# timwhite0/smcdet

Measured on AMD Instinct MI355X. Metric: particle-steps/sec (4096 particles, 32x32 tile), higher is better.
Workload: dtype f32

## Files before the change

smcdet_amd/csrc/mh_kernel.hip:

```cpp
#include <math.h>
#include <string.h>

#include <algorithm>
#include <cmath>
#include <mutex>
#include <type_traits>
#include <vector>

#include "mh_plan.h"
#include "render.h"
#include "tile.h"

namespace smcdet {

SMCDET_WAVE_TABLE

#ifdef SMCDET_DIAG
constexpr bool kDiag = true;
#else
constexpr bool kDiag = false;
#endif

constexpr int kMhBlock = kMhWaves * kWave;
constexpr int kSlots = 6;
constexpr int kBatch = 21;

struct MhArgs {
  DevModel m;
  DevPrior pr;
  int K, T, N, S;
  float sl, isl, sf, isf;
  float lb_h, lb_w, ub_h, ub_w;
  float lb_f, ub_f;
  uint32_t k0, k1;
  uint64_t offset;
  uint32_t ablate;
  int by_count;
  int scalar_slots;
  int skip_done;
  int no_psf_cache;
  int no_rcp_cache;
  int blk_slots;
  int generic_geometry;
  int no_write_through;
  int write_through;
  const float4* psf_tab;
  float tab_inv_h;
  const float* img;
  const float* temperature;
  const int64_t* ancestors;
  const float* anc_bins;
  const float* counts_in;
  const float* locs_in;
  const float* fluxes_in;
  float* counts_out;
  float* locs_out;
  float* fluxes_out;
  float* loglik_out;
  const float* rate_in;
  float* rate_out;
  const int32_t* go;
  const float* boxes;
  int32_t* acc_count;
  float* acc_rate;
  const int32_t* r_comp;
  const float* r_uloc;
  const float* r_uflux;
  const float* r_uacc;
  float* r_loga;
  uint8_t* r_accept;
  int has_tail;
  TileArgs tail;
};

constexpr int kTailMaxN = 8 * kTB;
static_assert(kMhPad == kWave && kMhMaxLdsPixels == kMaxLdsPixels && kMhTailMaxN == kTailMaxN &&
                  kMhTabFloats * sizeof(float) == kTabNodes * sizeof(float4),
              "mh_plan.h: constants out of step with device.h / tile.h");

__device__ __forceinline__ void tn_cache(float mu, float isig, float lb, float ub, float& phl,
                                         float& lZ) {
  phl = normal_cdf(lb, mu, isig);
  lZ = nan_to_num(fast_log(normal_cdf(ub, mu, isig) - phl), 0.0f);
}

__device__ __forceinline__ bool edge_hit(float hast) { return __float_as_uint(hast) == 0xff800000u; }

struct Proposal {
  int j;
  float h, w;
  float hn, wn, fn;
  float hast;
};

struct Dim {
  float sig, isig, lb, ub;
};

template <bool ABLATE>
__device__ __forceinline__ void propose_lane(float mu, float c_ph, float c_lZ, float u,
                                             const Dim& dm, float& xn, float& n_ph, float& n_lZ,
                                             float& hast_d, float& n_lf) {
  if (ABLATE) {
    xn = fminf(fmaxf(mu + (u - 0.5f) * dm.sig, dm.lb), dm.ub);
    n_ph = c_ph;
    n_lZ = c_lZ;
    hast_d = 0.f;
    n_lf = xn;
  } else {
    const float pc = fminf(fmaxf(u, 1e-6f), 0.999999f);
    float pt = c_ph + pc * fast_exp(c_lZ);
    pt = fminf(fmaxf(pt, 1e-6f), 0.999999f);
    xn = mu + dm.sig * erfinv_fast(2.0f * pt - 1.0f) * kSqrt2;
    xn = fminf(fmaxf(xn, dm.lb), dm.ub);
    tn_cache(xn, dm.isig, dm.lb, dm.ub, n_ph, n_lZ);
    hast_d = c_lZ - n_lZ;
    n_lf = fast_log(xn);
  }
}

template <int MODEL, bool WINDOWS, bool GL = false, bool RV = false, bool TB = false>
__device__ __forceinline__ float position_delta(const DevModel& m, const float* xs,
                                                const float* lg, const float* lam,
                                                const float* rv, const float4* tab, float tinv,
                                                int p, int aa, int bb, int ph, int pw,
                                                const Proposal& P, float amp_o, float amp_n,
                                                int ao_h, int ao_w, int an_h, int an_w,
                                                float& lnew, float& rnew) {
  const float fph = (float)ph + 0.5f, fpw = (float)pw + 0.5f;
  const float dho = fph - P.h, dwo = fpw - P.w;
  const float dhn = fph - P.hn, dwn = fpw - P.wn;
  float psi_o, psi_n;
  if constexpr (TB) {
    psi_o = psf_tab(tab, tinv, fmaf(dho, dho, dwo * dwo));
    psi_n = psf_tab(tab, tinv, fmaf(dhn, dhn, dwn * dwn));
  } else {
    psi_o = psf_raw<MODEL>(m, fmaf(dho, dho, dwo * dwo));
    psi_n = psf_raw<MODEL>(m, fmaf(dhn, dhn, dwn * dwn));
  }
  if (WINDOWS) {
    const unsigned span = 2u * (unsigned)m.R;
    psi_o = ((unsigned)(aa - ao_h) <= span && (unsigned)(bb - ao_w) <= span) ? psi_o : 0.f;
    psi_n = ((unsigned)(aa - an_h) <= span && (unsigned)(bb - an_w) <= span) ? psi_n : 0.f;
  }
  const float dl = fmaf(amp_n, psi_n, -amp_o * psi_o);
  const float lo = lam[p];
  lnew = lo + dl;
  const float lgx = (MODEL == SMCDET_MODEL_POISSON) ? lg[p] : 0.0f;
  const float x = GL ? xs[min(p, m.H * m.W - 1)] : xs[p];
  if constexpr (RV) {
    const float r0 = rv[p];
    const float v1 = fmaf(m.eta, lnew, m.s0sq);
    const float r1 = fast_rcp(v1);
    rnew = r1;
    const float d0 = x - lo, d1 = x - lnew;
    const float t = fmaf(d0 * d0, r0, -(d1 * d1) * r1);
    return fmaf(0.5f, t, (-0.5f * kLn2) * fast_log2(v1 * r0));
  }
  return pix_delta<MODEL>(m, x, lgx, lo, dl);
}

template <int MODEL, bool WINDOWS, bool GL = false, bool RV = false, bool TB = false>
__device__ __forceinline__ f2 position_delta2(const DevModel& m, const float* xs, const float* lg,
                                             const float* lam, const float* rv,
                                             const float4* tab, float tinv, const int (&p)[2],
                                             const int (&aa)[2], const int (&bb)[2], f2 fph,
                                             f2 fpw, const Proposal& P, float amp_o, float amp_n,
                                             int ao_h, int ao_w, int an_h, int an_w, f2& lnew,
                                             f2& rnew) {
  const f2 dho = fph - P.h, dwo = fpw - P.w;
  const f2 dhn = fph - P.hn, dwn = fpw - P.wn;
  f2 psi_o, psi_n;
  if constexpr (TB) {
    psi_o = psf_tab2(tab, tinv, fma2(dho, dho, dwo * dwo));
    psi_n = psf_tab2(tab, tinv, fma2(dhn, dhn, dwn * dwn));
  } else {
    psi_o = psf_raw2<MODEL>(m, fma2(dho, dho, dwo * dwo));
    psi_n = psf_raw2<MODEL>(m, fma2(dhn, dhn, dwn * dwn));
  }
  if (WINDOWS) {
    const unsigned span = 2u * (unsigned)m.R;
#pragma unroll
    for (int h = 0; h < 2; ++h) {
      psi_o[h] = ((unsigned)(aa[h] - ao_h) <= span && (unsigned)(bb[h] - ao_w) <= span) ? psi_o[h]
                                                                                       : 0.f;
      psi_n[h] = ((unsigned)(aa[h] - an_h) <= span && (unsigned)(bb[h] - an_w) <= span) ? psi_n[h]
                                                                                       : 0.f;
    }
  }
  const f2 dl = fma2(psi_n, amp_n, -amp_o * psi_o);
  const f2 lo = {lam[p[0]], lam[p[1]]};
  f2 x;
  if constexpr (GL) {
    const int hw1 = m.H * m.W - 1;
    x = f2{xs[min(p[0], hw1)], xs[min(p[1], hw1)]};
  } else {
    x = f2{xs[p[0]], xs[p[1]]};
  }
  lnew = lo + dl;
  if constexpr (RV) {
    const f2 r0 = {rv[p[0]], rv[p[1]]};
    const f2 v1 = fma2(lnew, m.eta, m.s0sq);
    const f2 r1 = rcp2(v1);
    rnew = r1;
    const f2 d0 = x - lo, d1 = x - lnew;
    const f2 t = fma2(d0 * d0, r0, -(d1 * d1) * r1);
    return fma2(t, 0.5f, (-0.5f * kLn2) * log2_2(v1 * r0));
  }
  f2 lgx = {0.f, 0.f};
  if constexpr (MODEL == SMCDET_MODEL_POISSON) lgx = f2{lg[p[0]], lg[p[1]]};
  return pix_delta2<MODEL>(m, x, lgx, lo, dl);
}

typedef float f4 __attribute__((ext_vector_type(4)));

template <int MODEL, bool RV>
__device__ __forceinline__ f2 delta_from_dl2(const DevModel& m, f2 x, f2 lo, f2 dl,
                                             const float* rv, const int (&p)[2], f2& lnew,
                                             f2& rnew) {
  lnew = lo + dl;
  if constexpr (RV) {
    const f2 r0 = {rv[p[0]], rv[p[1]]};
    const f2 v1 = fma2(lnew, m.eta, m.s0sq);
    const f2 r1 = rcp2(v1);
    rnew = r1;
    const f2 d0 = x - lo, d1 = x - lnew;
    const f2 t = fma2(d0 * d0, r0, -(d1 * d1) * r1);
    return fma2(t, 0.5f, (-0.5f * kLn2) * log2_2(v1 * r0));
  }
  return pix_delta2<MODEL>(m, x, f2{0.f, 0.f}, lo, dl);
}

template <int MODEL, bool WINDOWS, bool TB = false>
__device__ __forceinline__ float position_delta_pc(const DevModel& m, const float* xs,
                                                   const float* lg, const float* lam,
                                                   const float* pcj, const float4* tab,
                                                   float tinv, int p, bool valid, int aa,
                                                   int bb, int ph, int pw, const Proposal& P,
                                                   float amp_o, float amp_n, int an_h, int an_w,
                                                   float& lnew, float& psi_new) {
  const float fph = (float)ph + 0.5f, fpw = (float)pw + 0.5f;
  const float dhn = fph - P.hn, dwn = fpw - P.wn;
  const float psi_o = pcj[valid ? p : 0];
  float psi_n;
  if constexpr (TB) psi_n = psf_tab(tab, tinv, fmaf(dhn, dhn, dwn * dwn));
  else psi_n = psf_raw<MODEL>(m, fmaf(dhn, dhn, dwn * dwn));
  if (WINDOWS) {
    const unsigned span = 2u * (unsigned)m.R;
    psi_n = ((unsigned)(aa - an_h) <= span && (unsigned)(bb - an_w) <= span) ? psi_n : 0.f;
  }
  psi_new = psi_n;
  const float dl = fmaf(amp_n, psi_n, -amp_o * psi_o);
  const float lo = lam[p];
  lnew = lo + dl;
  const float lgx = (MODEL == SMCDET_MODEL_POISSON) ? lg[p] : 0.0f;
  return pix_delta<MODEL>(m, xs[p], lgx, lo, dl);
}

template <int PPL>
constexpr int rate_regs() { return 4 * ((PPL + 3) / 4); }
template <int PPL>
__device__ __forceinline__ void rate_load_regs(const float* __restrict__ rin,
                                               float (&r)[rate_regs<PPL>()], int HW, int lane) {
  constexpr int NV = (PPL + 3) / 4;
  if ((HW & 3) == 0) {
#pragma unroll
    for (int k = 0; k < NV; ++k) {
      const int p = 4 * (k * kWave + lane);
// ... 168 lines not shown
                        (PC ? kMhWaves * 10 * 1023 : 0) + 3) & ~3),
                  "the table's offset and mh_plan.h disagree");
    float4* t4 = reinterpret_cast<float4*>(smem + off);
    for (int i = threadIdx.x; i < kTabNodes; i += kMhBlock) t4[i] = a.psf_tab[i];
    tab = t4;
  }
  __syncthreads();
  SMC_TRACE(trow, 1);
  if (n >= a.N) return;

  const int N = a.N, S = a.S;
  size_t src;
  if constexpr (kHT) {
    src = a.ancestors ? (size_t)t * N + (size_t)anc_i : pid;
    if (a.anc_bins)
      src = (size_t)t * N +
            (size_t)bins_ancestor_from(a.anc_bins + (size_t)t * N, true, anc_b, N, anc_U, n);
  } else {
    src = a.ancestors ? (size_t)t * N + (size_t)a.ancestors[pid] : pid;
    if (a.anc_bins)
      src = (size_t)t * N +
            (size_t)bins_ancestor(a.anc_bins + (size_t)t * N,
                                  a.anc_bins + (size_t)a.T * (N + 1) + (size_t)t * kBinsCoarse, N,
                                  a.anc_bins[(size_t)a.T * N + t], n);
  }
  if constexpr (GL) lam = a.rate_out + pid * (size_t)HWp;
  float count_v = 0.f;
  if constexpr (kHT) count_v = a.counts_in[src];
  float sh = 0.f, sw = 0.f, sfx = 0.f;
  auto load_state = [&]() {
    if (lane < S) {
      sh = a.locs_in[(src * S + lane) * 2 + 0];
      sw = a.locs_in[(src * S + lane) * 2 + 1];
      sfx = a.fluxes_in[src * S + lane];
    }
  };
  [[maybe_unused]] float rate_r[rate_regs<(PPL > 0 ? PPL : 1)>()];
  if constexpr (kHT) {
    load_state();
    if constexpr (!FULL && !GL) {
      if (a.rate_in) rate_load_regs<PPL>(a.rate_in + src * (size_t)HW, rate_r, HW, lane);
    }
  } else {
    count_v = a.counts_in[src];
  }
  const float count = wave_uniform(count_v);
  if (a.counts_out && lane == 0) a.counts_out[pid] = count;
  const int Sj = a.by_count ? min(max((int)count, 0), S) : S;
  if constexpr (!kHT) tau_v = a.temperature[t];
  const float tau = wave_uniform(tau_v);
  const int K = (Sj > 0 && !(a.skip_done && tau >= 1.0f)) ? a.K : 0;
  if constexpr (!kHT) load_state();
  SMC_TRACE(trow, 2);

  [[maybe_unused]] float* rv = nullptr;
  if constexpr (RV) rv = lam + mh_lds_region(HWp);
  double cur_ll = 0.0;
  if constexpr (GL && !FULL) {
    if (a.rate_in && !(a.rate_in == a.rate_out && src == pid)) {
      const float* rin = a.rate_in + src * (size_t)HWp;
      for (int p = lane; p < HW; p += kWave) lam[p] = rin[p];
      wave_sync();
    } else if (!a.rate_in) {
      render_chunks<MODEL>(m, lam, sh, sw, sfx, S, lane);
    }
  } else if constexpr (GL) {
    render_sources<MODEL>(m, lam, sh, sw, sfx, S, lane);
    cur_ll = pixel_sum<MODEL>(m, xs, lg, lam, nullptr, lane);
  } else if constexpr (!FULL) {
    if (a.rate_in) {
      [[maybe_unused]] const float* rin = a.rate_in + src * (size_t)HW;
      if constexpr (PPL > 0) {
        if constexpr (!kHT) {
          rate_load_regs<PPL>(rin, rate_r, HW, lane);
          rate_store_lds<PPL, false>(m, rate_r, lam, nullptr, HW, lane);
          wave_sync();
        } else {
          rate_store_lds<PPL, RV>(m, rate_r, lam, rv, HW, lane);
        }
      } else if ((HW & 3) == 0) {
        for (int p = 4 * lane; p < HW; p += 4 * kWave) {
          const float4 v = *reinterpret_cast<const float4*>(rin + p);
          lam[p] = v.x;
          lam[p + 1] = v.y;
          lam[p + 2] = v.z;
          lam[p + 3] = v.w;
        }
      } else {
        for (int p = lane; p < HW; p += kWave) lam[p] = rin[p];
      }
      wave_sync();
    } else if constexpr (PPL > 0) {
      float lamk[PPL > 0 ? PPL : 1];
      render_regs<MODEL, PPL>(m, lamk, sh, sw, sfx, S, lane);
      store_regs<MODEL, PPL>(m, lam, lamk, lane);
    } else {
      render_sources<MODEL>(m, lam, sh, sw, sfx, S, lane);
    }
  } else if constexpr (PPL > 0) {
    float lamk[PPL > 0 ? PPL : 1];
    render_regs<MODEL, PPL>(m, lamk, sh, sw, sfx, S, lane);
    cur_ll = pixel_sum_regs<MODEL, PPL>(m, xs, lg, lamk, lane);
  } else {
    render_sources<MODEL>(m, lam, sh, sw, sfx, S, lane);
    cur_ll = pixel_sum<MODEL>(m, xs, lg, lam, nullptr, lane);
  }
  lam[HW + lane] = m.bg;
  auto row_off = [&](int ph) -> int {
    if constexpr (GEO::kFixed) return ph * GEO::kW;
    else return (int)__umul24((unsigned)ph, (unsigned)m.W);
  };
  [[maybe_unused]] const float* rv_rd = nullptr;
  if constexpr (RV) {
    rv_rd = GEO::kFixed ? lam + mh_lds_region(a.m.H * a.m.W + kWave) : rv;
    wave_sync();
    if (kHT && a.rate_in) {
      rv[HW + lane] = fast_rcp(fmaf(m.eta, m.bg, m.s0sq));
    } else if constexpr (PPL > 0) {
      constexpr int NR = PPL + 1;
      float v[NR];
#pragma unroll
      for (int k = 0; k < NR; ++k) {
        const int p = k * kWave + lane;
        v[k] = p < HWp ? lam[p] : 0.f;
      }
#pragma unroll
      for (int k = 0; k < NR; ++k) {
        const int p = k * kWave + lane;
        if (p < HWp) rv[p] = fast_rcp(fmaf(m.eta, v[k], m.s0sq));
      }
    } else {
      for (int p = lane; p < HWp; p += kWave) rv[p] = fast_rcp(fmaf(m.eta, lam[p], m.s0sq));
    }
    wave_sync();
  }
  [[maybe_unused]] float* pcw = nullptr;
  if constexpr (PC) {
    pcw = smem + mh_lds_cache(kImg, HWp) + wave * S * HW;
    const int ph = lane / m.W, pw = lane - ph * m.W;
    const float fph = (float)ph + 0.5f, fpw = (float)pw + 0.5f;
    for (int s = 0; s < S; ++s) {
      const float hs = readlane(sh, s), ws = readlane(sw, s);
      const int fh = ifloor16(hs), fw = ifloor16(ws);
      const float dh = fph - hs, dw = fpw - ws;
      float v;
      if constexpr (TB) v = psf_tab(tab, tinv, fmaf(dh, dh, dw * dw));
      else v = psf_raw<MODEL>(m, fmaf(dh, dh, dw * dw));
      if (lane < HW) pcw[s * HW + lane] = (abs(ph - fh) <= m.R && abs(pw - fw) <= m.R) ? v : 0.f;
    }
    wave_sync();
  }
  SMC_TRACE(trow, 3);

  const int lb3 = lane / 3;
  const int d = lane - 3 * lb3;
  Dim dm;
  dm.isig = d < 2 ? a.isl : a.isf;
  dm.sig = d < 2 ? a.sl : a.sf;
  {
    float lb_h = a.lb_h, lb_w = a.lb_w, ub_h = a.ub_h, ub_w = a.ub_w;
    if (a.boxes) {
      const float* bx_ = a.boxes + 4 * t;
      lb_h = bx_[0];
      lb_w = bx_[1];
      ub_h = bx_[2];
      ub_w = bx_[3];
    }
    dm.lb = d == 0 ? lb_h : (d == 1 ? lb_w : a.lb_f);
    dm.ub = d == 0 ? ub_h : (d == 1 ? ub_w : a.ub_f);
  }
  const bool ablate_prop = kDiag && (a.ablate & SMCDET_MH_ABLATE_PROPOSAL) != 0;
  const bool ablate_lik = kDiag && (a.ablate & SMCDET_MH_ABLATE_LIKELIHOOD) != 0;

  float ru0 = 0.f, ru1 = 0.f, ru2 = 0.f, ru3 = 0.f, ru4 = 0.f;
  int rcomp = 0;
  auto refill = [&](int k0) {
    const int kk = k0 + lane;
    if constexpr (REPLAY) {
      if (kk < a.K) {
        const size_t r = ((size_t)kk * a.T + t) * N + n;
        rcomp = a.r_comp[r];
        ru1 = a.r_uloc[r * 2 + 0];
        ru2 = a.r_uloc[r * 2 + 1];
        ru3 = a.r_uflux[r];
        ru4 = a.r_uacc[r];
      }
    } else {
      const uint64_t ctr = a.offset + (uint64_t)kk;
      const uint32_t c0 = (uint32_t)ctr, c1 = (uint32_t)(ctr >> 32);
      const U4 r0 = philox4x32(c0, c1, (uint32_t)pid, kTagMH0, a.k0, a.k1);
      const U4 r1 = philox4x32(c0, c1, (uint32_t)pid, kTagMH1, a.k0, a.k1);
      ru0 = u01(r0.x);
      ru1 = u01(r0.y);
      ru2 = u01(r0.z);
      ru3 = u01(r0.w);
      ru4 = u01(r1.x);
    }
  };

  float bx = 0.f, bhd = 0.f;
  float bmu = 0.f, bampo = 0.f, bampn = 0.f, bdp = 0.f, bhs = 0.f, blu = 0.f;
  int bfl = 0;
  unsigned bmg = 1u;
  int bj = 0, batch_k0 = 0, batch_n = 0;
  uint64_t dirty = 0;
  auto compute_batch = [&](int k0) {
    const int n_ = min(min(kBatch, kWave - (k0 & 63)), K - k0);
    const int b = min(lb3, n_ - 1);
    const int kl = (k0 & 63) + b;
    int j;
    if constexpr (REPLAY) j = __shfl(rcomp, kl, kWave);
    else j = min((int)(__shfl(ru0, kl, kWave) * (float)Sj), Sj - 1);
    const float u1 = __shfl(ru1, kl, kWave), u2 = __shfl(ru2, kl, kWave);
    const float u3 = __shfl(ru3, kl, kWave);
    const float u = d == 0 ? u1 : (d == 1 ? u2 : u3);
    const float m0 = __shfl(sh, j, kWave), m1 = __shfl(sw, j, kWave), m2 = __shfl(sfx, j, kWave);
    const float mu = d == 0 ? m0 : (d == 1 ? m1 : m2);
    float c_ph, c_lZ;
    tn_cache(mu, dm.isig, dm.lb, dm.ub, c_ph, c_lZ);
    float n_ph, n_lZ, blf;
    if (ablate_prop)
      propose_lane<true>(mu, c_ph, c_lZ, u, dm, bx, n_ph, n_lZ, bhd, blf);
    else
      propose_lane<false>(mu, c_ph, c_lZ, u, dm, bx, n_ph, n_lZ, bhd, blf);
    bmu = mu;
    bfl = (int)(((unsigned)ifloor16(mu) & 0xffffu) | ((unsigned)ifloor16(bx) << 16));
    {
      const int f0 = ifloor16(mu), f1 = ifloor16(bx);
      const int c0_ = max(min(f0, f1) - m.R, 0), c1_ = min(max(f0, f1) + m.R, m.W - 1);
      const unsigned bw_ = (unsigned)max(c1_ - c0_ + 1, 1);
      bmg = (65536u + bw_ - 1u) / bw_;
    }
    const float lf_cur = fast_log(mu);
    bampo = m.g * mu * psf_scale<MODEL>(m);
    bampn = m.g * bx * psf_scale<MODEL>(m);
    bdp = ((float)j < count) ? flux_prior_delta<FP>(a.pr, mu, bx, lf_cur, blf) : 0.0f;
    if (d < 2 && bx >= dm.ub) bhd = -INFINITY;
    const float hd0 = __shfl(bhd, max(lane - 2, 0), kWave);
    const float hd1 = __shfl(bhd, max(lane - 1, 0), kWave);
    bhs = (hd0 + hd1 + bhd) + bdp;
    blu = fast_log(__shfl(ru4, kl, kWave));
    bj = j;
    batch_k0 = k0;
    batch_n = n_;
    dirty = 0;
  };

  int accept = 0;
#ifdef SMCDET_TRACE
  unsigned tr_pos = 0, tr_acc = 0;
#endif
  __builtin_amdgcn_s_setprio(3);
  bool frozen = false;
  int k = 0;
  for (int q = 0; q < 4 && !frozen; ++q) {
    if (q == 1) __builtin_amdgcn_s_setprio(2);
    else if (q == 2) __builtin_amdgcn_s_setprio(1);
    else if (q == 3) __builtin_amdgcn_s_setprio(0);
    const int kend = ((q + 1) * K + 3) >> 2;
    for (; k < kend; ++k) {
    const int kl = k & 63;
    if (kl == 0) refill(k);
    if (k >= batch_k0 + batch_n) compute_batch(k);
    int b = k - batch_k0;
    int j = readlane(bj, 3 * b);
    if ((dirty >> j) & 1ull) {
      compute_batch(k);
      b = 0;
      j = readlane(bj, 0);
    }
    const int b3 = __builtin_amdgcn_readfirstlane(3 * b);
    Proposal P;
    P.j = j;
    P.h = readlane(bmu, b3);
    P.w = readlane(bmu, b3 + 1);
    P.hn = readlane(bx, b3);
    P.wn = readlane(bx, b3 + 1);
    P.fn = readlane(bx, b3 + 2);
    P.hast = readlane(bhs, b3 + 2);
    const float log_u = readlane(blu, b3 + 2);
    const float amp_o = readlane(bampo, b3 + 2), amp_n = readlane(bampn, b3 + 2);

    float dll;
    double new_ll = 0.0;
    float s_lam[NSL];
    int s_pix[NSL];
    [[maybe_unused]] float s_rv[RV ? NSL : 1];
    [[maybe_unused]] float s_psi = 0.f;
    int npos = 0, bw = 1, r0 = 0, c0 = 0, nslots = 0;
    if constexpr (FULL) {
      const float ch = lane == P.j ? P.hn : sh, cw = lane == P.j ? P.wn : sw;
      const float cf = lane == P.j ? P.fn : sfx;
      if constexpr (PPL > 0) {
        float lamk[PPL > 0 ? PPL : 1];
        render_regs<MODEL, PPL>(m, lamk, ch, cw, cf, S, lane);
        new_ll = pixel_sum_regs<MODEL, PPL>(m, xs, lg, lamk, lane);
      } else {
        render_sources<MODEL>(m, lam, ch, cw, cf, S, lane);
        new_ll = pixel_sum<MODEL>(m, xs, lg, lam, nullptr, lane);
      }
      dll = (float)(new_ll - cur_ll);
    } else {
      const int flh = readlane(bfl, b3), flw = readlane(bfl, b3 + 1);
      const int fh0 = (int)(int16_t)(flh & 0xffff), fh1 = flh >> 16;
      const int fw0 = (int)(int16_t)(flw & 0xffff), fw1 = flw >> 16;
      r0 = max(min(fh0, fh1) - m.R, 0);
      const int r1 = min(max(fh0, fh1) + m.R, m.H - 1);
      c0 = max(min(fw0, fw1) - m.R, 0);
      const int c1 = min(max(fw0, fw1) + m.R, m.W - 1);
      bw = c1 - c0 + 1;
      npos = (r1 >= r0 && c1 >= c0 && !ablate_lik) ? (r1 - r0 + 1) * bw : 0;
      nslots = (npos + kWave - 1) / kWave;
#ifdef SMCDET_TRACE
      tr_pos += npos;
#endif
      const unsigned magic = (unsigned)readlane((int)bmg, b3 + 1);
      const bool same = (fh0 == fh1) && (fw0 == fw1);
      const int ao_h = fh0 - m.R - r0, ao_w = fw0 - m.R - c0;
      const int an_h = fh1 - m.R - r0, an_w = fw1 - m.R - c0;
      auto slots = [&](auto NS, auto WIN) -> float {
        constexpr int ns = decltype(NS)::value;
        constexpr bool win = decltype(WIN)::value;
        float acc = 0.f;
#pragma unroll
        for (int i = 0; i < ns; ++i) {
          const int q = i * kWave + lane;
          const bool valid = q < npos;
          const int aa = (int)(__umul24((unsigned)q, magic) >> 16);
          const int bb = q - (int)__umul24((unsigned)aa, (unsigned)bw);
          const int ph = r0 + aa, pw = c0 + bb;
          const int p = valid ? row_off(ph) + pw : HW + lane;
          float lnew, rnew, e;
          if constexpr (PC)
            e = position_delta_pc<MODEL, win, TB>(m, xs, lg, lam, pcw + P.j * HW, tab, tinv, p,
                                                  valid, aa, bb, ph, pw, P, amp_o, amp_n, an_h,
                                                  an_w, lnew, s_psi);
          else
            e = position_delta<MODEL, win, GL, RV, TB>(m, xs, lg, lam, rv, tab, tinv, p, aa, bb,
                                                       ph, pw, P, amp_o, amp_n, ao_h, ao_w, an_h,
                                                       an_w, lnew, rnew);
          acc += valid ? e : 0.f;
          s_lam[i] = lnew;
          if constexpr (RV) s_rv[i] = rnew;
          s_pix[i] = p;
        }
        return acc;
      };
      auto pairs = [&](auto NP, auto ODD, auto WIN) -> float {
        constexpr int np = decltype(NP)::value;
        constexpr bool odd = decltype(ODD)::value;
        constexpr bool win = decltype(WIN)::value;
        f2 acc = {0.f, 0.f};
#pragma unroll
        for (int i = 0; i < np; ++i) {
          int aa[2], bb[2], p[2];
          bool valid[2];
          f2 fph, fpw;
#pragma unroll
          for (int h = 0; h < 2; ++h) {
            const int q = (2 * i + h) * kWave + lane;
            valid[h] = q < npos;
            aa[h] = (int)(__umul24((unsigned)q, magic) >> 16);
            bb[h] = q - (int)__umul24((unsigned)aa[h], (unsigned)bw);
            const int ph = r0 + aa[h], pw = c0 + bb[h];
            p[h] = valid[h] ? row_off(ph) + pw : HW + lane;
            fph[h] = (float)ph + 0.5f;
            fpw[h] = (float)pw + 0.5f;
          }
          f2 lnew, rnew;
          f2 e = position_delta2<MODEL, win, GL, RV, TB>(m, xs, lg, lam, rv_rd, tab, tinv, p, aa,
                                                         bb, fph, fpw, P, amp_o, amp_n, ao_h, ao_w,
                                                         an_h, an_w, lnew, rnew);
          e.x = valid[0] ? e.x : 0.f;
          e.y = valid[1] ? e.y : 0.f;
          acc += e;
          s_lam[2 * i] = lnew.x;
          s_lam[2 * i + 1] = lnew.y;
          if constexpr (RV) {
            s_rv[2 * i] = rnew.x;
            s_rv[2 * i + 1] = rnew.y;
          }
          s_pix[2 * i] = p[0];
          s_pix[2 * i + 1] = p[1];
        }
        float acc1 = 0.f;
        if constexpr (odd) {
          const int q = 2 * np * kWave + lane;
          const bool valid = q < npos;
          const int aa = (int)(__umul24((unsigned)q, magic) >> 16);
          const int bb = q - (int)__umul24((unsigned)aa, (unsigned)bw);
          const int ph = r0 + aa, pw = c0 + bb;
          const int p = valid ? row_off(ph) + pw : HW + lane;
          float lnew, rnew;
          const float e = position_delta<MODEL, win, GL, RV, TB>(m, xs, lg, lam, rv, tab, tinv, p,
                                                             aa, bb, ph, pw, P, amp_o, amp_n,
                                                             ao_h, ao_w, an_h, an_w, lnew, rnew);
          acc1 = valid ? e : 0.f;
          s_lam[2 * np] = lnew;
          if constexpr (RV) s_rv[2 * np] = rnew;
          s_pix[2 * np] = p;
        }
        return (acc.x + acc.y) + acc1;
      };
      using I0 = std::integral_constant<int, 0>;
      using I1 = std::integral_constant<int, 1>;
      using One = std::true_type;
      using Zero = std::false_type;
      using I2 = std::integral_constant<int, 2>;
      using I3 = std::integral_constant<int, 3>;
      using I4 = std::integral_constant<int, 4>;
      using I5 = std::integral_constant<int, 5>;
      using I8 = std::integral_constant<int, kSlots>;
      using Win = std::true_type;
      using Same = std::false_type;
      auto far_positions = [&](auto WRITE) -> float {
        float acc = 0.f;
        const float inv_bw = 1.0f / (float)bw;
        for (int q = kSlots * kWave + lane; q < npos; q += kWave) {
          const int aa = (int)(((float)q + 0.5f) * inv_bw);
          const int bb = q - (int)__umul24((unsigned)aa, (unsigned)bw);
          const int ph = r0 + aa, pw = c0 + bb;
          const int p = row_off(ph) + pw;
          float lnew, rnew;
          acc += position_delta<MODEL, true, GL, RV, TB>(m, xs, lg, lam, rv, tab, tinv, p, aa, bb,
                                                         ph, pw, P, amp_o, amp_n, ao_h, ao_w, an_h,
                                                         an_w, lnew, rnew);
          if constexpr (decltype(WRITE)::value) {
            lam[p] = lnew;
            if constexpr (RV) rv[p] = rnew;
          }
        }
        return acc;
      };
      auto finish = [&](float dsum, auto NS) {
        constexpr int ns = decltype(NS)::value;
        constexpr bool kFar = NSL > 1 && ns >= kSlots;
        if (kFar && npos > kSlots * kWave) dsum += far_positions(std::false_type{});
        dll = wave_sum(dsum);
        accept = __builtin_amdgcn_ballot_w64(fmaf(tau, dll, P.hast) >= log_u) != 0;
        if (accept && !edge_hit(P.hast)) {
#pragma unroll
          for (int i = 0; i < ns; ++i)
            if (i < nslots) {
              lam[s_pix[i]] = s_lam[i];
              if constexpr (RV) rv[s_pix[i]] = s_rv[i];
            }
          if (kFar && npos > kSlots * kWave) (void)far_positions(std::true_type{});
          wave_sync();
        }
      };
      constexpr bool kBlk = MODEL == SMCDET_MODEL_M71 && PPL > 1 && !GL && !TB && PAIRED;
      bool blk = false;
      if constexpr (kBlk)
        blk = same && a.blk_slots > 0 && m.R <= 8 && nslots >= a.blk_slots && r1 - r0 >= 15 &&
              c1 - c0 >= 15 && r1 - r0 <= 16 && c1 - c0 <= 16;
      auto block = [&]() -> float {
        const int li = lane & 15, lk = lane >> 4;
        const bool knew = lk < 2;
        const float kk = (lk & 1) ? m.k2 : m.k1;
        const float ak = (knew ? amp_n : -amp_o) * ((lk & 1) ? m.b : 1.0f);
        const float dy = ((float)(r0 + li) + 0.5f) - (knew ? P.hn : P.h);
        const float dx = ((float)(c0 + li) + 0.5f) - (knew ? P.wn : P.w);
        const float av = ak * fast_exp2(kk * (dy * dy));
        const float bv = fast_exp2(kk * (dx * dx));
        const f4 g = __builtin_amdgcn_mfma_f32_16x16x4f32(av, bv, f4{0.f, 0.f, 0.f, 0.f}, 0, 0, 0);
        const int prow0 = r0 + 4 * lk, pcol = c0 + li;
        const float fpw = (float)pcol + 0.5f;
        const float dwo = fpw - P.w, dwn = fpw - P.wn;
        const f2 dwo2 = {dwo * dwo, dwo * dwo}, dwn2 = {dwn * dwn, dwn * dwn};
        const float po = amp_o * m.p0, pn = amp_n * m.p0;
        const int pb = prow0 * m.W + pcol;
        const float fph0 = (float)prow0 + 0.5f;
        f2 acc = {0.f, 0.f};
#pragma unroll
        for (int h = 0; h < 2; ++h) {
          const f2 fph = {fph0 + (float)(2 * h), fph0 + (float)(2 * h + 1)};
          const f2 dho = fph - P.h, dhn = fph - P.hn;
          const f2 e3o = exp2_2(m.kb * log2_2(fma2(fma2(dho, dho, dwo2), m.k3, 1.0f)));
          const f2 e3n = exp2_2(m.kb * log2_2(fma2(fma2(dhn, dhn, dwn2), m.k3, 1.0f)));
          const f2 dl = f2{g[2 * h], g[2 * h + 1]} + fma2(e3n, pn, -po * e3o);
          const int p[2] = {pb + 2 * h * m.W, pb + (2 * h + 1) * m.W};
          const f2 lo = {lam[p[0]], lam[p[1]]};
          const f2 x = {xs[p[0]], xs[p[1]]};
          f2 lnew, rnew;
          acc += delta_from_dl2<MODEL, RV>(m, x, lo, dl, rv, p, lnew, rnew);
          s_lam[2 * h] = lnew.x;
          s_lam[2 * h + 1] = lnew.y;
          s_pix[2 * h] = p[0];
          s_pix[2 * h + 1] = p[1];
          if constexpr (RV) {
            s_rv[2 * h] = rnew.x;
            s_rv[2 * h + 1] = rnew.y;
          }
        }
        const int nb = r1 > r0 + 15 ? c1 - c0 + 1 : 0;
        const int nr = c1 > c0 + 15 ? 16 : 0;
        const bool valid = lane < nb + nr, bot = lane < nb;
        const int ph = bot ? r0 + 16 : r0 + (lane - nb);
        const int pw = bot ? c0 + lane : c0 + 16;
        const int p = valid ? ph * m.W + pw : HW + lane;
        float lnew, rnew;
        const float e = position_delta<MODEL, false, false, RV, false>(
            m, xs, lg, lam, rv, tab, tinv, p, 0, 0, ph, pw, P, amp_o, amp_n, 0, 0, 0, 0, lnew, rnew);
        s_lam[4] = lnew;
        s_pix[4] = p;
        if constexpr (RV) s_rv[4] = rnew;
        return (acc.x + acc.y) + (valid ? e : 0.f);
      };
      if constexpr (NSL == 1) {
        float dsum = 0.f;
        if (nslots == 1) dsum = same ? slots(I1{}, Same{}) : slots(I1{}, Win{});
        dll = wave_sum(dsum);
        accept = __builtin_amdgcn_ballot_w64(fmaf(tau, dll, P.hast) >= log_u) != 0;
      } else if (blk) {
        if constexpr (kBlk) {
          nslots = 5;
          finish(block(), I5{});
        }
      } else if (nslots == 0) {
        finish(0.f, I0{});
      } else if (PAIRED && nslots == 1) {
        if (same) finish(pairs(I0{}, One{}, Same{}), I1{});
        else finish(pairs(I0{}, One{}, Win{}), I1{});
      } else if (PAIRED && nslots == 2) {
        if (same) finish(pairs(I1{}, Zero{}, Same{}), I2{});
        else finish(pairs(I1{}, Zero{}, Win{}), I2{});
      } else if (PAIRED && nslots <= 3) {
        if (same) finish(pairs(I1{}, One{}, Same{}), I3{});
        else finish(pairs(I1{}, One{}, Win{}), I3{});
      } else if (PAIRED && nslots <= 4) {
        if (same) finish(pairs(I2{}, Zero{}, Same{}), I4{});
        else finish(pairs(I2{}, Zero{}, Win{}), I4{});
      } else if (PAIRED && nslots <= 5) {
        if (same) finish(pairs(I2{}, One{}, Same{}), I5{});
        else finish(pairs(I2{}, One{}, Win{}), I5{});
      } else if (PAIRED) {
        finish(slots(I8{}, Win{}), I8{});
      } else if (nslots <= 3) {
        if (same) finish(slots(I3{}, Same{}), I3{});
        else finish(slots(I3{}, Win{}), I3{});
      } else if (nslots <= 5) {
        if (same) finish(slots(I5{}, Same{}), I5{});
        else finish(slots(I5{}, Win{}), I5{});
      } else {
        finish(slots(I8{}, Win{}), I8{});
      }
    }
    if constexpr (FULL) {
      const float loga = fmaf(tau, dll, P.hast);
      accept = __builtin_amdgcn_readfirstlane((loga >= log_u) ? 1 : 0);
    }
#ifdef SMCDET_TRACE
    tr_acc += accept;
#endif
    if constexpr (REPLAY) {
      if (lane == 0) {
        const size_t r = ((size_t)k * a.T + t) * N + n;
        if (a.r_loga) a.r_loga[r] = fmaf(tau, dll, P.hast);
        if (a.r_accept) a.r_accept[r] = (uint8_t)(accept && P.hast != -INFINITY);
      }
    }
    if (edge_hit(P.hast)) {
      frozen = true;
      break;
    }
    if (accept) {
      if constexpr (FULL) {
        cur_ll = new_ll;
      } else {
        if constexpr (NSL == 1) {
          if (nslots == 1) {
            lam[s_pix[0]] = s_lam[0];
            if constexpr (PC)
              if (s_pix[0] < HW) pcw[P.j * HW + s_pix[0]] = s_psi;
          }
          wave_sync();
        }
        cur_ll += (double)dll;
      }
      sh = writelane(P.hn, P.j, sh);
      sw = writelane(P.wn, P.j, sw);
      sfx = writelane(P.fn, P.j, sfx);
      dirty |= 1ull << P.j;
    }
    }
  }

  __builtin_amdgcn_s_setprio(0);
  SMC_TRACE(trow, 4);
#ifdef SMCDET_TRACE
  SMC_WAVE_STAT(trow, 5, tr_pos);
  SMC_WAVE_STAT(trow, 6, tr_acc);
#endif
  if (lane < S) {
    a.locs_out[(pid * S + lane) * 2 + 0] = sh;
    a.locs_out[(pid * S + lane) * 2 + 1] = sw;
    a.fluxes_out[pid * S + lane] = sfx;
  }
  auto store_rate = [&]() {
    if constexpr (!FULL && !GL) {
      if (a.rate_out) {
        float* rout = a.rate_out + pid * (size_t)HW;
        if constexpr (kHT) {
          const char* kp = (const char*)__builtin_amdgcn_kernarg_segment_ptr();
          __asm__ volatile("" : "+s"(kp));
          const bool wt =
              *reinterpret_cast<const int*>(kp + offsetof(MhArgs, write_through)) != 0;
          wave_sync();
          copy_out_regs<PPL>(lam, rout, HW, lane, wt);
        } else if constexpr (PPL > 0) {
          copy_out_regs<PPL>(lam, rout, HW, lane, false);
        } else if ((HW & 3) == 0) {
          for (int p = 4 * lane; p < HW; p += 4 * kWave)
            *reinterpret_cast<float4*>(rout + p) = make_float4(lam[p], lam[p + 1], lam[p + 2],
                                                               lam[p + 3]);
        } else {
          for (int p = lane; p < HW; p += kWave) rout[p] = lam[p];
        }
      }
    }
  };
  if constexpr (kHT) store_rate();
  if (a.loglik_out) {
    double ll;
    if constexpr (!FULL) {
      ll = pixel_sum<MODEL>(m, xs, lg, lam, nullptr, lane);
    } else if constexpr (PPL > 0) {
      float lamk[PPL > 0 ? PPL : 1];
      render_regs<MODEL, PPL>(m, lamk, sh, sw, sfx, S, lane);
      ll = pixel_sum_regs<MODEL, PPL>(m, xs, lg, lamk, lane);
    } else {
      render_sources<MODEL>(m, lam, sh, sw, sfx, S, lane);
      ll = pixel_sum<MODEL>(m, xs, lg, lam, nullptr, lane);
    }
    if (lane == 0) a.loglik_out[pid] = (float)ll;
  }
  if constexpr (!kHT) store_rate();
  SMC_TRACE(trow, 5);
  SMC_WAVE_MARK(trow, 1);
  if constexpr (TAIL) __threadfence();
  if (lane == 0) {
    const int nw = min(kMhWaves, N - (int)blockIdx.x * kMhWaves);
    if (accept && a.K > 0) atomicAdd(&wg_acc, 1);
    __threadfence_block();
    if (atomicAdd(&wg_done, 1) == nw - 1) {
      unsigned long long* slot = reinterpret_cast<unsigned long long*>(a.acc_count) + t;
      const unsigned long long mine = (unsigned long long)(unsigned)atomicAdd(&wg_acc, 0);
      const unsigned long long old = atomicAdd(slot, (mine << 32) | 1ull);
      if ((unsigned)(old & 0xffffffffull) == gridDim.x - 1) {
        const unsigned long long total = (old >> 32) + mine;
        atomicExch(slot, 0ull);
        a.acc_rate[t] = (float)total / (float)N;
        wg_last = 1;
      }
    }
  }
  if constexpr (TAIL && PPL != 1 && !FULL && PAIRED) {
    {
      __shared__ TileRed tail_red;
      __syncthreads();
      if (wg_last) {
        __builtin_amdgcn_fence(__ATOMIC_ACQUIRE, "agent");
        const TileArgs* tp = reinterpret_cast<const TileArgs*>(
            (const char*)__builtin_amdgcn_kernarg_segment_ptr() +
            offsetof(MhArgs, tail));
        __asm__ volatile("" : "+s"(tp));
        tile_work<kMhBlock, 8>(*tp, t, smem, tail_red, -1);
      }
    }
  }
}

using MhKernel = void (*)(MhArgs);

template <bool REPLAY, bool FULL, int PPL>
static MhKernel mh_kernel_normal_of(const MhPlan& p) {
  constexpr int M = SMCDET_MODEL_POISSON;
  constexpr bool kInc = !FULL;
  switch (p.variant) {
    case kMhPC:
      if constexpr (kInc && PPL == 1)
        return mh_sweep_kernel<M, REPLAY, FULL, PPL, true, false, false, true, false, false,
                               GeoRun, kFluxNormal>;
      break;
    case kMhTail:
      if constexpr (kInc && PPL != 1)
        return mh_sweep_kernel<M, REPLAY, FULL, PPL, true, true, false, false, false, false,
                               GeoRun, kFluxNormal>;
      break;
    case kMhPaired:
      if constexpr (kInc)
        return mh_sweep_kernel<M, REPLAY, FULL, PPL, true, false, false, false, false, false,
                               GeoRun, kFluxNormal>;
      break;
    case kMhUnpaired:
      if constexpr (FULL)
        return mh_sweep_kernel<M, REPLAY, FULL, PPL, false, false, false, false, false, false,
                               GeoRun, kFluxNormal>;
      break;
    default:
      break;
  }
  return nullptr;
}

template <bool REPLAY, bool FULL>
static MhKernel mh_kernel_normal_at(const MhPlan& p) {
  return p.ppl == 1    ? mh_kernel_normal_of<REPLAY, FULL, 1>(p)
         : p.ppl == 4  ? mh_kernel_normal_of<REPLAY, FULL, 4>(p)
         : p.ppl == 16 ? mh_kernel_normal_of<REPLAY, FULL, 16>(p)
                       : mh_kernel_normal_of<REPLAY, FULL, 0>(p);
}

static MhKernel mh_kernel_normal_for(const MhPlan& p, bool replay, bool full) {
  if (replay) return full ? mh_kernel_normal_at<true, true>(p) : mh_kernel_normal_at<true, false>(p);
  return full ? mh_kernel_normal_at<false, true>(p) : mh_kernel_normal_at<false, false>(p);
}

template <int MODEL, bool REPLAY, bool FULL, int PPL>
static MhKernel mh_kernel_of(const MhPlan& p) {
  constexpr bool kM71 = MODEL == SMCDET_MODEL_M71, kInc = !FULL;
  constexpr bool kReg = kM71 && kInc && PPL > 1;
  switch (p.variant) {
    case kMhPCTB:
      if constexpr (kDiag && kM71 && kInc && PPL == 1)
        return mh_sweep_kernel<MODEL, REPLAY, FULL, PPL, true, false, false, true, false, true>;
      break;
    case kMhPC:
      if constexpr (kInc && PPL == 1)
        return mh_sweep_kernel<MODEL, REPLAY, FULL, PPL, true, false, false, true>;
      break;
    case kMhRVTB:
      if constexpr (kDiag && kReg)
        return mh_sweep_kernel<MODEL, REPLAY, FULL, PPL, true, false, false, false, true, true>;
      break;
    case kMhTB:
      if constexpr (kDiag && kM71 && kInc && PPL > 0)
        return mh_sweep_kernel<MODEL, REPLAY, FULL, PPL, true, false, false, false, false, true>;
      break;
    case kMhRV:
      if constexpr (kReg && PPL == 16) {
        if (p.geo_fixed)
          return mh_sweep_kernel<MODEL, REPLAY, FULL, PPL, true, false, false, false, true, false,
                                 GeoFixed<32, 32, 8>>;
      }
// ... 406 lines not shown
```

smcdet_amd/csrc/mh_plan.h:

```cpp
#pragma once
#include <stddef.h>
#include <stdint.h>

#include "../../include/smcdet_hip.h"

#ifdef __HIP__
#define SMCDET_HD __host__ __device__
#else
#define SMCDET_HD
#endif
#ifndef SMCDET_SMALL_TILE_WAVES
#define SMCDET_SMALL_TILE_WAVES 7
#endif

namespace smcdet {
constexpr int kMhWaves = 4;
constexpr int kMhPad = 64;
constexpr int kMhMaxLdsPixels = 4096;
constexpr int kMhTailMaxN = 4096;
constexpr int kMhTabFloats = 4 * 513;
constexpr size_t kMhLdsPerCu = 160 * 1024;

SMCDET_HD constexpr int mh_lds_rates(int imgs, int HWp) { return imgs * HWp; }
SMCDET_HD constexpr int mh_lds_region(int HWp) { return kMhWaves * HWp; }
SMCDET_HD constexpr int mh_lds_cache(int imgs, int HWp) { return (imgs + kMhWaves) * HWp; }
SMCDET_HD constexpr int mh_lds_floats(int imgs, int HWp, int HW, int S, bool rv, bool pc) {
  return mh_lds_cache(imgs, HWp) + (rv ? mh_lds_region(HWp) : 0) + (pc ? kMhWaves * S * HW : 0);
}
SMCDET_HD constexpr int mh_lds_tab(int imgs, int HWp, int HW, int S, bool rv, bool pc) {
  return (mh_lds_floats(imgs, HWp, HW, S, rv, pc) + 3) & ~3;
}
constexpr size_t mh_lds_bytes(int model, int HW, int S, bool rv, bool pc, bool tab) {
  const int imgs = model == SMCDET_MODEL_POISSON ? 2 : 1, HWp = HW + kMhPad;
  return sizeof(float) * (size_t)(tab ? mh_lds_tab(imgs, HWp, HW, S, rv, pc) + kMhTabFloats
                                      : mh_lds_floats(imgs, HWp, HW, S, rv, pc));
}
constexpr int mh_wg_per_cu(int ppl, bool replay, bool full) {
  return ppl == 1 ? (replay ? SMCDET_SMALL_TILE_WAVES - 1 : SMCDET_SMALL_TILE_WAVES)
                  : (full && ppl == 16 ? 2 : 4);
}

enum MhVariant {
  kMhGL,
  kMhPC,
  kMhPaired,
  kMhRV,
  kMhTail,
  kMhUnpaired,
  kMhTB, kMhPCTB, kMhRVTB
};
enum MhTailMode { kMhNoTail, kMhTailFused, kMhTailSplit };

struct MhPlanIn {
  int model, H, W, R;
  int N, S, T;
  uint32_t flags;
  bool tail;
  size_t tail_lds;
  bool diag;
  bool replay = false, two_launch = false;
  bool rate_out = false;
  bool psf_tab = false;
  int cu_count = 0;
};
struct MhPlan {
  int status = SMCDET_OK;
  const char* msg = "";
  int ppl = 0;
  MhVariant variant = kMhPaired;
  bool geo_fixed = false;
  size_t lds = 0;
  MhTailMode tail = kMhNoTail;
  bool write_through = false;
};

inline MhPlan mh_plan(const MhPlanIn& in) {
  MhPlan p;
  const bool m71 = in.model == SMCDET_MODEL_M71, full = in.flags & SMCDET_MH_FULL_RECOMPUTE;
  const bool scalar = in.diag && (in.flags & SMCDET_MH_SCALAR_SLOTS), paired = !full && !scalar;
  const bool no_pc = in.flags & SMCDET_MH_NO_PSF_CACHE;
  const long long HW = (long long)in.H * in.W;
  auto lds = [&](bool rv, bool pc, bool tab) {
    return mh_lds_bytes(in.model, (int)HW, in.S, rv, pc, tab);
  };
  if (HW > kMhMaxLdsPixels) {
    static_assert(kMhMaxLdsPixels == 4096, "the message names it");
    if (scalar)
      return {SMCDET_EUNSUPPORTED, "tiles above 4096 pixels: no fused step / scalar slots"};
    p.variant = kMhGL;
    p.tail = in.tail ? kMhTailSplit : kMhNoTail;
    return p;
  }
  if (in.S <= kMhPad) p.ppl = HW <= 64 ? 1 : HW <= 256 ? 4 : HW <= 1024 ? 16 : 0;
  p.lds = lds(false, false, false);
  if (in.tail) {
    const size_t need = p.lds > in.tail_lds ? p.lds : in.tail_lds;
    const bool fusable = !(in.flags & (SMCDET_MH_FULL_RECOMPUTE | SMCDET_MH_SCALAR_SLOTS)) &&
                         in.N % kMhWaves == 0 && in.N <= kMhTailMaxN && p.ppl != 1 &&
                         4 * (need + 2048) <= kMhLdsPerCu;
    p.tail = fusable && !in.two_launch ? kMhTailFused : kMhTailSplit;
    if (p.tail == kMhTailFused) p.lds = need;
  }
  const bool fused = p.tail == kMhTailFused;
  if (fused && (!paired || p.ppl == 1)) return {SMCDET_EINVAL, "fused step: unsupported shape"};
  p.write_through = p.ppl > 1 && !full && !fused && in.rate_out &&
                    !(in.flags & SMCDET_MH_NO_WRITE_THROUGH) &&
                    (long long)((in.N + kMhWaves - 1) / kMhWaves) * in.T <=
                        (long long)in.cu_count * mh_wg_per_cu(p.ppl, in.replay, full);
  auto take = [&](bool on, MhVariant v, bool rv, bool pc, bool tab, int wg_per_cu) {
    if (!on || (size_t)wg_per_cu * (lds(rv, pc, tab) + 1024) > kMhLdsPerCu) return false;
    p.variant = v;
    p.lds = lds(rv, pc, tab);
    return true;
  };
  const bool tb = in.diag && in.psf_tab && m71 && paired && !fused;
  if (p.ppl == 1 && !full) {
    constexpr int wg = SMCDET_SMALL_TILE_WAVES;
    if (take(tb && !no_pc, kMhPCTB, false, true, true, wg) ||
        take(paired && !no_pc, kMhPC, false, true, false, wg) ||
        take(tb, kMhTB, false, false, true, wg))
      return p;
  } else if (m71 && p.ppl > 1 && !full) {
    const bool rv = paired && !fused && !(in.diag && (in.flags & SMCDET_MH_NO_RCP_CACHE));
    if (take(tb && rv, kMhRVTB, true, false, true, 4) || take(tb, kMhTB, false, false, true, 4))
      return p;
    if (take(rv, kMhRV, true, false, false, 4)) {
      p.geo_fixed = p.ppl == 16 && in.H == 32 && in.W == 32 && in.R == 8 &&
                    !(in.flags & SMCDET_MH_GENERIC_GEOMETRY);
      return p;
    }
    if (!in.diag && !fused) return {SMCDET_EUNSUPPORTED, "M71 sweep: the 1/v image does not fit"};
  }
  p.variant = fused ? kMhTail : paired ? kMhPaired : kMhUnpaired;
  return p;
}
}
```

Baseline: 1.890 billion.

## Split truncated-normal proposal across lane pairs and precompute draw terms at refill

For multi-pixel-per-lane sweeps, each proposal dimension now uses two lanes. Each lane evaluates one bound's normal CDF and exchanges it with its partner via DPP, which halves the per-lane CDF work but makes each batch cover 10 entries instead of 21. The component index, the clamping of the uniforms and log(u_acc) move into refill, so they are done once per 64 draws. The integer division for the window magic is replaced with a float reciprocal plus correction. Trace counters for batches and rebatches are also added.

```diff
diff --git a/smcdet_amd/csrc/mh_kernel.hip b/smcdet_amd/csrc/mh_kernel.hip
--- a/smcdet_amd/csrc/mh_kernel.hip
+++ b/smcdet_amd/csrc/mh_kernel.hip
@@ -95,6 +95,7 @@
 
 struct Dim {
   float sig, isig, lb, ub;
+  float bd;
 };
 
 template <bool ABLATE>
@@ -114,6 +115,34 @@
     xn = mu + dm.sig * erfinv_fast(2.0f * pt - 1.0f) * kSqrt2;
     xn = fminf(fmaxf(xn, dm.lb), dm.ub);
     tn_cache(xn, dm.isig, dm.lb, dm.ub, n_ph, n_lZ);
+    hast_d = c_lZ - n_lZ;
+    n_lf = fast_log(xn);
+  }
+}
+
+__device__ __forceinline__ void tn_cache_pair(float mu, const Dim& dm, bool side, float& phl,
+                                              float& lZ) {
+  const float mine = normal_cdf(dm.bd, mu, dm.isig);
+  const float other = dpp_f<0xb1>(mine);
+  phl = side ? other : mine;
+  lZ = nan_to_num(fast_log((side ? mine : other) - phl), 0.0f);
+}
+
+template <bool ABLATE>
+__device__ __forceinline__ void propose_pair(float mu, float pc, const Dim& dm, bool side,
+                                             float& xn, float& hast_d, float& n_lf) {
+  if (ABLATE) {
+    xn = fminf(fmaxf(mu + (pc - 0.5f) * dm.sig, dm.lb), dm.ub);
+    hast_d = 0.f;
+    n_lf = xn;
+  } else {
+    float c_ph, c_lZ, n_ph, n_lZ;
+    tn_cache_pair(mu, dm, side, c_ph, c_lZ);
+    float pt = c_ph + pc * fast_exp(c_lZ);
+    pt = fminf(fmaxf(pt, 1e-6f), 0.999999f);
+    xn = mu + dm.sig * erfinv_fast(2.0f * pt - 1.0f) * kSqrt2;
+    xn = fminf(fmaxf(xn, dm.lb), dm.ub);
+    tn_cache_pair(xn, dm, side, n_ph, n_lZ);
     hast_d = c_lZ - n_lZ;
     n_lf = fast_log(xn);
   }
@@ -588,8 +617,14 @@
   }
   SMC_TRACE(trow, 3);
 
-  const int lb3 = lane / 3;
-  const int d = lane - 3 * lb3;
+  constexpr bool kSix = PPL > 1 && !FULL;
+  constexpr int kEntryLanes = kSix ? 6 : 3;
+  constexpr int kDimLanes = kSix ? 2 : 1;
+  constexpr bool kDrawTerms = kSix;
+  constexpr int kEntries = kSix ? 10 : kBatch;
+  const int lb3 = lane / kEntryLanes;
+  const int d = kSix ? (lane - kEntryLanes * lb3) >> 1 : lane - 3 * lb3;
+  [[maybe_unused]] const bool side = (lane & 1) != 0;
   Dim dm;
   dm.isig = d < 2 ? a.isl : a.isf;
   dm.sig = d < 2 ? a.sl : a.sf;
@@ -604,6 +639,7 @@
     }
     dm.lb = d == 0 ? lb_h : (d == 1 ? lb_w : a.lb_f);
     dm.ub = d == 0 ? ub_h : (d == 1 ? ub_w : a.ub_f);
+    dm.bd = side ? dm.ub : dm.lb;
   }
   const bool ablate_prop = kDiag && (a.ablate & SMCDET_MH_ABLATE_PROPOSAL) != 0;
   const bool ablate_lik = kDiag && (a.ablate & SMCDET_MH_ABLATE_LIKELIHOOD) != 0;
@@ -632,6 +668,15 @@
       ru3 = u01(r0.w);
       ru4 = u01(r1.x);
     }
+    if constexpr (kDrawTerms) {
+      if constexpr (!REPLAY) rcomp = min((int)(ru0 * (float)Sj), Sj - 1);
+      if (!ablate_prop) {
+        ru1 = fminf(fmaxf(ru1, 1e-6f), 0.999999f);
+        ru2 = fminf(fmaxf(ru2, 1e-6f), 0.999999f);
+        ru3 = fminf(fmaxf(ru3, 1e-6f), 0.999999f);
+      }
+      ru4 = fast_log(ru4);
+    }
   };
 
   float bx = 0.f, bhd = 0.f;
@@ -640,42 +685,58 @@
   unsigned bmg = 1u;
   int bj = 0, batch_k0 = 0, batch_n = 0;
   uint64_t dirty = 0;
+#ifdef SMCDET_TRACE
+  unsigned tr_bat = 0, tr_reb = 0, tr_it = 0, tr_long = 0;
+#endif
   auto compute_batch = [&](int k0) {
-    const int n_ = min(min(kBatch, kWave - (k0 & 63)), K - k0);
+#ifdef SMCDET_TRACE
+    ++tr_bat;
+    if (batch_n > 0 && k0 - batch_k0 >= 10) ++tr_long;
+#endif
+    const int n_ = min(min(kEntries, kWave - (k0 & 63)), K - k0);
     const int b = min(lb3, n_ - 1);
     const int kl = (k0 & 63) + b;
     int j;
-    if constexpr (REPLAY) j = __shfl(rcomp, kl, kWave);
+    if constexpr (REPLAY || kDrawTerms) j = __shfl(rcomp, kl, kWave);
     else j = min((int)(__shfl(ru0, kl, kWave) * (float)Sj), Sj - 1);
     const float u1 = __shfl(ru1, kl, kWave), u2 = __shfl(ru2, kl, kWave);
     const float u3 = __shfl(ru3, kl, kWave);
     const float u = d == 0 ? u1 : (d == 1 ? u2 : u3);
     const float m0 = __shfl(sh, j, kWave), m1 = __shfl(sw, j, kWave), m2 = __shfl(sfx, j, kWave);
     const float mu = d == 0 ? m0 : (d == 1 ? m1 : m2);
-    float c_ph, c_lZ;
-    tn_cache(mu, dm.isig, dm.lb, dm.ub, c_ph, c_lZ);
-    float n_ph, n_lZ, blf;
-    if (ablate_prop)
-      propose_lane<true>(mu, c_ph, c_lZ, u, dm, bx, n_ph, n_lZ, bhd, blf);
-    else
-      propose_lane<false>(mu, c_ph, c_lZ, u, dm, bx, n_ph, n_lZ, bhd, blf);
+    float blf;
+    if constexpr (kSix) {
+      if (ablate_prop) propose_pair<true>(mu, u, dm, side, bx, bhd, blf);
+      else propose_pair<false>(mu, kDrawTerms ? u : fminf(fmaxf(u, 1e-6f), 0.999999f), dm, side, bx,
+                               bhd, blf);
+    } else {
+      float c_ph, c_lZ;
+      tn_cache(mu, dm.isig, dm.lb, dm.ub, c_ph, c_lZ);
+      float n_ph, n_lZ;
+      if (ablate_prop)
+        propose_lane<true>(mu, c_ph, c_lZ, u, dm, bx, n_ph, n_lZ, bhd, blf);
+      else
+        propose_lane<false>(mu, c_ph, c_lZ, u, dm, bx, n_ph, n_lZ, bhd, blf);
+    }
     bmu = mu;
     bfl = (int)(((unsigned)ifloor16(mu) & 0xffffu) | ((unsigned)ifloor16(bx) << 16));
     {
       const int f0 = ifloor16(mu), f1 = ifloor16(bx);
       const int c0_ = max(min(f0, f1) - m.R, 0), c1_ = min(max(f0, f1) + m.R, m.W - 1);
       const unsigned bw_ = (unsigned)max(c1_ - c0_ + 1, 1);
-      bmg = (65536u + bw_ - 1u) / bw_;
+      if constexpr (kSix) bmg = mh_window_magic(bw_, fast_rcp((float)bw_));
+      else bmg = (65536u + bw_ - 1u) / bw_;
     }
     const float lf_cur = fast_log(mu);
     bampo = m.g * mu * psf_scale<MODEL>(m);
     bampn = m.g * bx * psf_scale<MODEL>(m);
     bdp = ((float)j < count) ? flux_prior_delta<FP>(a.pr, mu, bx, lf_cur, blf) : 0.0f;
     if (d < 2 && bx >= dm.ub) bhd = -INFINITY;
-    const float hd0 = __shfl(bhd, max(lane - 2, 0), kWave);
-    const float hd1 = __shfl(bhd, max(lane - 1, 0), kWave);
+    const float hd0 = __shfl(bhd, max(lane - 2 * kDimLanes, 0), kWave);
+    const float hd1 = __shfl(bhd, max(lane - kDimLanes, 0), kWave);
     bhs = (hd0 + hd1 + bhd) + bdp;
-    blu = fast_log(__shfl(ru4, kl, kWave));
+    if constexpr (kDrawTerms) blu = __shfl(ru4, kl, kWave);
+    else blu = fast_log(__shfl(ru4, kl, kWave));
     bj = j;
     batch_k0 = k0;
     batch_n = n_;
@@ -699,23 +760,27 @@
     if (kl == 0) refill(k);
     if (k >= batch_k0 + batch_n) compute_batch(k);
     int b = k - batch_k0;
-    int j = readlane(bj, 3 * b);
+    int j = readlane(bj, kEntryLanes * b);
     if ((dirty >> j) & 1ull) {
+#ifdef SMCDET_TRACE
+      ++tr_reb;
+#endif
       compute_batch(k);
       b = 0;
       j = readlane(bj, 0);
     }
-    const int b3 = __builtin_amdgcn_readfirstlane(3 * b);
+    const int b3 = __builtin_amdgcn_readfirstlane(kEntryLanes * b);
     Proposal P;
     P.j = j;
     P.h = readlane(bmu, b3);
-    P.w = readlane(bmu, b3 + 1);
+    P.w = readlane(bmu, b3 + kDimLanes);
     P.hn = readlane(bx, b3);
-    P.wn = readlane(bx, b3 + 1);
-    P.fn = readlane(bx, b3 + 2);
-    P.hast = readlane(bhs, b3 + 2);
-    const float log_u = readlane(blu, b3 + 2);
-    const float amp_o = readlane(bampo, b3 + 2), amp_n = readlane(bampn, b3 + 2);
+    P.wn = readlane(bx, b3 + kDimLanes);
+    P.fn = readlane(bx, b3 + 2 * kDimLanes);
+    P.hast = readlane(bhs, b3 + 2 * kDimLanes);
+    const float log_u = readlane(blu, b3 + 2 * kDimLanes);
+    const float amp_o = readlane(bampo, b3 + 2 * kDimLanes),
+                amp_n = readlane(bampn, b3 + 2 * kDimLanes);
 
     float dll;
     double new_ll = 0.0;
@@ -737,7 +802,7 @@
       }
       dll = (float)(new_ll - cur_ll);
     } else {
-      const int flh = readlane(bfl, b3), flw = readlane(bfl, b3 + 1);
+      const int flh = readlane(bfl, b3), flw = readlane(bfl, b3 + kDimLanes);
       const int fh0 = (int)(int16_t)(flh & 0xffff), fh1 = flh >> 16;
       const int fw0 = (int)(int16_t)(flw & 0xffff), fw1 = flw >> 16;
       r0 = max(min(fh0, fh1) - m.R, 0);
@@ -750,7 +815,7 @@
 #ifdef SMCDET_TRACE
       tr_pos += npos;
 #endif
-      const unsigned magic = (unsigned)readlane((int)bmg, b3 + 1);
+      const unsigned magic = (unsigned)readlane((int)bmg, b3 + kDimLanes);
       const bool same = (fh0 == fh1) && (fw0 == fw1);
       const int ao_h = fh0 - m.R - r0, ao_w = fw0 - m.R - c0;
       const int an_h = fh1 - m.R - r0, an_w = fw1 - m.R - c0;
@@ -988,6 +1053,7 @@
     }
 #ifdef SMCDET_TRACE
     tr_acc += accept;
+    ++tr_it;
 #endif
     if constexpr (REPLAY) {
       if (lane == 0) {
@@ -1025,8 +1091,11 @@
   __builtin_amdgcn_s_setprio(0);
   SMC_TRACE(trow, 4);
 #ifdef SMCDET_TRACE
-  SMC_WAVE_STAT(trow, 5, tr_pos);
-  SMC_WAVE_STAT(trow, 6, tr_acc);
+  SMC_WAVE_STAT(trow, 5, (unsigned long long)tr_pos | (unsigned long long)tr_long << 32);
+  SMC_WAVE_STAT(trow, 6,
+                (unsigned long long)(tr_acc & 0xffffu) | (unsigned long long)(tr_reb & 0xffffu) << 16 |
+                    (unsigned long long)(tr_bat & 0xffffu) << 32 |
+                    (unsigned long long)(tr_it & 0xffffu) << 48);
 #endif
   if (lane < S) {
     a.locs_out[(pid * S + lane) * 2 + 0] = sh;
diff --git a/smcdet_amd/csrc/mh_plan.h b/smcdet_amd/csrc/mh_plan.h
--- a/smcdet_amd/csrc/mh_plan.h
+++ b/smcdet_amd/csrc/mh_plan.h
@@ -34,6 +34,12 @@
   const int imgs = model == SMCDET_MODEL_POISSON ? 2 : 1, HWp = HW + kMhPad;
   return sizeof(float) * (size_t)(tab ? mh_lds_tab(imgs, HWp, HW, S, rv, pc) + kMhTabFloats
                                       : mh_lds_floats(imgs, HWp, HW, S, rv, pc));
+}
+SMCDET_HD inline unsigned mh_window_magic(unsigned bw, float rcp_bw) {
+  const float fbw = (float)bw;
+  const float q0 = __builtin_truncf(65536.0f * rcp_bw);
+  const float r = 65536.0f - q0 * fbw;
+  return (unsigned)q0 + (unsigned)(r > 0.0f) + (unsigned)(r > fbw);
 }
 constexpr int mh_wg_per_cu(int ppl, bool replay, bool full) {
   return ppl == 1 ? (replay ? SMCDET_SMALL_TILE_WAVES - 1 : SMCDET_SMALL_TILE_WAVES)
```

After: 1.885 billion. No clear change (-0.3%).
